# Wuziyi616/multi_part_assembly

Measured on AMD Instinct MI355X. Metric: train-step parts/sec (BxP) at N=1000 pts, higher is better.
Workload: dtype f32

## Files before the change

multi_part_assembly_amd/csrc/pn_bwd_q.h:

```cpp

#ifdef PN_TIMING
#define PN_T_DECL unsigned long long t_busy = 0, t_mark = __builtin_amdgcn_s_memtime(), t_start = t_mark;
#define PN_BAR                                         \
  {                                                    \
    t_busy += __builtin_amdgcn_s_memtime() - t_mark;   \
    __syncthreads();                                   \
    t_mark = __builtin_amdgcn_s_memtime();             \
  }
#define PN_T_REPORT(ROLE)                                                                                              \
  if (blockIdx.x == 5 && lane == 0)                                                                                    \
    printf("K=%d FIRST=%d %s wave %d: units %d busy %llu of %llu cycles\n", K, (int)FIRST, ROLE, wave, n_it, t_busy, \
           __builtin_amdgcn_s_memtime() - t_start);
#else
#define PN_T_DECL
#define PN_BAR __syncthreads();
#define PN_T_REPORT(ROLE)
#endif
#define PN_LDS __attribute__((address_space(3)))
typedef short pn_s16x4 __attribute__((ext_vector_type(4)));
typedef short pn_s16x8 __attribute__((ext_vector_type(8)));
typedef unsigned int pn_u32x4 __attribute__((ext_vector_type(4)));

__device__ __forceinline__ pn_bf16x8 pn_tr_frag(const unsigned char* p, int stride) {
  const pn_s16x4 a = __builtin_amdgcn_ds_read_tr16_b64_v4i16((PN_LDS pn_s16x4*)p);
  const pn_s16x4 b = __builtin_amdgcn_ds_read_tr16_b64_v4i16((PN_LDS pn_s16x4*)(p + 4 * stride));
  const pn_s16x8 v = {a[0], a[1], a[2], a[3], b[0], b[1], b[2], b[3]};
  return __builtin_bit_cast(pn_bf16x8, v);
}

__device__ __forceinline__ void pn_split4(const float v[4], pn_bf16x4& ph, pn_bf16x4& pm, pn_bf16x4& pl) {
#pragma unroll
  for (int u = 0; u < 4; ++u) {
    ph[u] = (__bf16)v[u];
    const float r1 = v[u] - (float)ph[u];
    pm[u] = (__bf16)r1;
    pl[u] = (__bf16)(r1 - (float)pm[u]);
  }
}

typedef float pn_f32x2 __attribute__((ext_vector_type(2)));
typedef __bf16 pn_bf16x2 __attribute__((ext_vector_type(2)));
__device__ __forceinline__ void pn_split2v(pn_f32x2 x, pn_bf16x2& h, pn_bf16x2& m, pn_bf16x2& l) {
  h = __builtin_convertvector(x, pn_bf16x2);
  const pn_f32x2 r = x - __builtin_convertvector(h, pn_f32x2);
  m = __builtin_convertvector(r, pn_bf16x2);
  const pn_f32x2 t = r - __builtin_convertvector(m, pn_f32x2);
  l = __builtin_convertvector(t, pn_bf16x2);
}
__device__ __forceinline__ void pn_split4v(pn_f32x2 a, pn_f32x2 b, pn_bf16x4& ph, pn_bf16x4& pm, pn_bf16x4& pl) {
  pn_bf16x2 h0, m0, l0, h1, m1, l1;
  pn_split2v(a, h0, m0, l0);
  pn_split2v(b, h1, m1, l1);
  ph = pn_bf16x4{h0[0], h0[1], h1[0], h1[1]};
  pm = pn_bf16x4{m0[0], m0[1], m1[0], m1[1]};
  pl = pn_bf16x4{l0[0], l0[1], l1[0], l1[1]};
}

__device__ __forceinline__ void pn_fmac(float& acc, float a, float b) {
  asm volatile("v_fmac_f32 %0, %1, %2" : "+v"(acc) : "v"(a), "v"(b));
}

#define PN_MFMA6(ACC, AH, AM, AL, BH, BM, BL)                          \
  ACC = __builtin_amdgcn_mfma_f32_32x32x16_bf16(AH, BH, ACC, 0, 0, 0); \
  ACC = __builtin_amdgcn_mfma_f32_32x32x16_bf16(AH, BM, ACC, 0, 0, 0); \
  ACC = __builtin_amdgcn_mfma_f32_32x32x16_bf16(AM, BH, ACC, 0, 0, 0); \
  ACC = __builtin_amdgcn_mfma_f32_32x32x16_bf16(AM, BM, ACC, 0, 0, 0); \
  ACC = __builtin_amdgcn_mfma_f32_32x32x16_bf16(AH, BL, ACC, 0, 0, 0); \
  ACC = __builtin_amdgcn_mfma_f32_32x32x16_bf16(AL, BH, ACC, 0, 0, 0);

__global__ void pn_bwd_q_prep_kernel(const float* __restrict__ w, const float* __restrict__ coef, int K, int CIN,
                                     float* __restrict__ q) {
  const int k = blockIdx.x, d = threadIdx.x;
  float acc = 0.0f;
  if (k < CIN) {
#pragma unroll 8
    for (int c = 0; c < K; ++c) acc = __builtin_fmaf(coef[K + c] * w[(long long)c * CIN + k], w[(long long)c * CIN + d], acc);
  } else {
#pragma unroll 8
    for (int c = 0; c < K; ++c) acc = __builtin_fmaf(coef[2 * K + c], w[(long long)c * CIN + d], acc);
  }
  q[(long long)k * CIN + d] = acc;
}

__host__ __device__ constexpr int pn_bwd_q_elems(int K, int CIN, bool first) {
  return K * CIN + CIN * CIN + CIN + (first ? 192 + 12 : 0);
}

template <int N, typename F>
__device__ __forceinline__ void pn_static_for(F&& f) {
  if constexpr (N > 0) {
    pn_static_for<N - 1>(f);
    f(std::integral_constant<int, N - 1>{});
  }
}

struct PnWTile {
  signed char a, b, kind, orow, ocol;
};
template <int K>
struct PnWPlan;
template <>
struct PnWPlan<64> {
  static constexpr int TPW = 2;
  static constexpr PnWTile t[4][2] = {{{0, 8, 0, 0, 0}, {8, 8, 1, 0, 0}},
                                      {{0, 9, 0, 0, 1}, {8, 9, 1, 0, 1}},
                                      {{1, 8, 0, 1, 0}, {-1, -1, 0, 0, 0}},
                                      {{1, 9, 0, 1, 1}, {9, 9, 1, 1, 1}}};
  static constexpr int zc[4] = {0, 0, 1, 1};
  static constexpr bool uses(int w, int code) {
    for (int i = 0; i < TPW; ++i)
      if (t[w][i].a >= 0 && (t[w][i].a == code || t[w][i].b == code)) return true;
    return false;
  }
};
template <>
struct PnWPlan<128> {
  static constexpr int TPW = 3;
  static constexpr PnWTile t[4][3] = {{{0, 8, 0, 0, 0}, {0, 9, 0, 0, 1}, {8, 8, 1, 0, 0}},
                                      {{1, 8, 0, 1, 0}, {1, 9, 0, 1, 1}, {8, 9, 1, 0, 1}},
                                      {{2, 8, 0, 2, 0}, {2, 9, 0, 2, 1}, {9, 9, 1, 1, 1}},
                                      {{3, 8, 0, 3, 0}, {3, 9, 0, 3, 1}, {-1, -1, 0, 0, 0}}};
  static constexpr int zc[4] = {0, 1, 2, 3};
  static constexpr bool uses(int w, int code) {
    for (int i = 0; i < TPW; ++i)
      if (t[w][i].a >= 0 && (t[w][i].a == code || t[w][i].b == code)) return true;
    return false;
  }
};

template <int K, int CIN, int RB, int NS, int ND, int NW, bool FIRST, int KPN = 1>
__global__ __launch_bounds__(64 * (NS + ND + NW), (NS + ND + NW + 3) / 4) void pn_bwd_q_kernel(
    const float* __restrict__ dz, const float* __restrict__ y_prev, const float* __restrict__ bn_prev,
    const float* __restrict__ w, const float* __restrict__ coef, const float* __restrict__ q,
    const int* __restrict__ vlist, int N, float* __restrict__ dz_prev, float* __restrict__ partial,
    float* __restrict__ dwpart, const float* __restrict__ wt1) {
  constexpr int SZ = 6 * K + 16, SA = 6 * CIN + 16;
  constexpr int RT = RB / 32, CT = CIN / 32;
  constexpr int KZ = K / 16, KA = CIN / 16, KW = RB / 16;
  constexpr int NTS = 64 * NS, QK = K / 4, QC = CIN / 4, RG = NTS / QC;
  constexpr int NLZ = RB * QK / NTS, NLY = RB * QC / NTS;
  constexpr int ELEMS = pn_bwd_q_elems(K, CIN, FIRST);
  constexpr int OUTP = RB * CIN;
  static_assert(ND == RT * CT * KPN && RB * QK % NTS == 0 && RB * QC % NTS == 0 && NTS % QK == 0 && NTS % QC == 0, "shapes");
  static_assert(!FIRST || CIN == 64, "the recomputed input is the 64-channel first layer");
  __shared__ __attribute__((aligned(16))) unsigned char pz[2][RB * SZ];
  __shared__ __attribute__((aligned(16))) unsigned char pa[2][RB * SA];
  __shared__ __attribute__((aligned(16))) unsigned char wl[CIN * SZ];
  __shared__ __attribute__((aligned(16))) float outp[2][KPN][OUTP];
  const int wave = __builtin_amdgcn_readfirstlane(threadIdx.x >> 6), lane = threadIdx.x & 63, j = lane & 31, hh = lane >> 5;
  const int TB = (N + RB - 1) / RB, U = vlist[0] * TB, G = gridDim.x;
  const int n_it = (int)blockIdx.x < U ? (U - (int)blockIdx.x + G - 1) / G : 0;
  auto part_of = [&](int it) {
    const int u = (int)blockIdx.x + it * G;
    return u < U && it >= 0 ? vlist[4 + u / TB] : 0;
  };
  auto n0_of = [&](int it) { return (((int)blockIdx.x + it * G) % TB) * RB; };

  for (int e = threadIdx.x; e < CIN * (K / 4); e += blockDim.x) {
    const int d = e % CIN, k4 = e / CIN;
    float v[4];
#pragma unroll
    for (int u = 0; u < 4; ++u) v[u] = coef[4 * k4 + u] * w[(long long)(4 * k4 + u) * CIN + d];
    pn_bf16x4 ph, pm, pl;
    pn_split4(v, ph, pm, pl);
    unsigned char* p = wl + d * SZ + 8 * k4;
    *reinterpret_cast<pn_bf16x4*>(p) = ph;
    *reinterpret_cast<pn_bf16x4*>(p + 2 * K) = pm;
    *reinterpret_cast<pn_bf16x4*>(p + 4 * K) = pl;
  }

  static_assert(NW == NS && ND == NS && NLY % 2 == 0, "the epilogue uses the stagers' thread -> (row, 4 columns) map in both roles");
  constexpr int EH = NLY / 2;
    const int te = threadIdx.x & (NTS - 1);
    const int cy4 = te % QC, ry0 = te / QC;
    const float4 sc = reinterpret_cast<const float4*>(bn_prev)[cy4];
    const float4 sh = reinterpret_cast<const float4*>(bn_prev + CIN)[cy4];
    const float4 mn = reinterpret_cast<const float4*>(bn_prev + 2 * CIN)[cy4];
    float4 w1a = {}, w1b = {}, w1c = {};
    if constexpr (FIRST) {
      w1a = reinterpret_cast<const float4*>(wt1)[cy4];
      w1b = reinterpret_cast<const float4*>(wt1 + 64)[cy4];
      w1c = reinterpret_cast<const float4*>(wt1 + 128)[cy4];
    }
    auto first4 = [&](float4 p) {
      return make_float4(first_layer_y(p.x, p.y, p.z, w1a.x, w1b.x, w1c.x), first_layer_y(p.x, p.y, p.z, w1a.y, w1b.y, w1c.y),
                         first_layer_y(p.x, p.y, p.z, w1a.z, w1b.z, w1c.z), first_layer_y(p.x, p.y, p.z, w1a.w, w1b.w, w1c.w));
    };
    float4 ye[EH];
    float4 s1v = make_float4(0.0f, 0.0f, 0.0f, 0.0f), t2v = s1v;
    float4 sax = s1v, say = s1v, saz = s1v;
    auto load_y = [&](int it, int m, auto half_tag) {
      constexpr int HALF = decltype(half_tag)::value;
      const int n0 = n0_of(it);
      const long long row0 = (long long)m * N + n0;
#pragma unroll
      for (int i = 0; i < EH; ++i) {
        const int rl = ry0 + (HALF * EH + i) * RG;
        const int rr = n0 + rl < N ? rl : N - 1 - n0;
        if constexpr (FIRST) {
          const float* p = y_prev + (row0 + rr) * 3;
          ye[i] = make_float4(p[0], p[1], p[2], 0.0f);
        } else {
          ye[i] = reinterpret_cast<const float4*>(y_prev)[(row0 + rr) * QC + cy4];
        }
      }
    };
    auto epilogue = [&](int it, int m, auto half_tag) {
      constexpr int HALF = decltype(half_tag)::value;
      const int n0 = n0_of(it);
      const long long row0 = (long long)m * N + n0;
      const float* ob = &outp[it & 1][0][0];
#pragma unroll
      for (int i = 0; i < EH; ++i) {
        const int rl = ry0 + (HALF * EH + i) * RG;
        const bool ok = n0 + rl < N;
        float4 o = *reinterpret_cast<const float4*>(ob + rl * CIN + 4 * cy4);
        if constexpr (KPN == 2) {
          const float4 o2 = *reinterpret_cast<const float4*>(ob + OUTP + rl * CIN + 4 * cy4);
          o.x += o2.x;
          o.y += o2.y;
          o.z += o2.z;
          o.w += o2.w;
        }
        float4 yv = ye[i];
        float px = 0.0f, py = 0.0f, pzc = 0.0f;
        if constexpr (FIRST) {
          px = yv.x;
          py = yv.y;
          pzc = yv.z;
          yv = first4(yv);
        }
        float4 d;
        d.x = (ok && __builtin_fmaf(yv.x, sc.x, sh.x) > 0.0f) ? o.x : 0.0f;
        d.y = (ok && __builtin_fmaf(yv.y, sc.y, sh.y) > 0.0f) ? o.y : 0.0f;
        d.z = (ok && __builtin_fmaf(yv.z, sc.z, sh.z) > 0.0f) ? o.z : 0.0f;
        d.w = (ok && __builtin_fmaf(yv.w, sc.w, sh.w) > 0.0f) ? o.w : 0.0f;
        if constexpr (FIRST) {
          sax.x = __builtin_fmaf(d.x, px, sax.x);
          sax.y = __builtin_fmaf(d.y, px, sax.y);
          sax.z = __builtin_fmaf(d.z, px, sax.z);
          sax.w = __builtin_fmaf(d.w, px, sax.w);
          say.x = __builtin_fmaf(d.x, py, say.x);
          say.y = __builtin_fmaf(d.y, py, say.y);
          say.z = __builtin_fmaf(d.z, py, say.z);
          say.w = __builtin_fmaf(d.w, py, say.w);
          saz.x = __builtin_fmaf(d.x, pzc, saz.x);
          saz.y = __builtin_fmaf(d.y, pzc, saz.y);
          saz.z = __builtin_fmaf(d.z, pzc, saz.z);
          saz.w = __builtin_fmaf(d.w, pzc, saz.w);
        } else {
          if (ok) reinterpret_cast<float4*>(dz_prev)[(row0 + rl) * QC + cy4] = d;
        }
        s1v.x += d.x;
        s1v.y += d.y;
        s1v.z += d.z;
        s1v.w += d.w;
        t2v.x = __builtin_fmaf(d.x, yv.x - mn.x, t2v.x);
        t2v.y = __builtin_fmaf(d.y, yv.y - mn.y, t2v.y);
        t2v.z = __builtin_fmaf(d.z, yv.z - mn.z, t2v.z);
        t2v.w = __builtin_fmaf(d.w, yv.w - mn.w, t2v.w);
      }
    };
    auto put_sums = [&](int role) {
      float* scr = reinterpret_cast<float*>(&pz[0][0]);
      const float* isd = bn_prev + 3 * CIN;
      asm volatile("" : "+s"(isd));
      const float4 is4 = reinterpret_cast<const float4*>(isd)[cy4];
      t2v.x *= is4.x;
      t2v.y *= is4.y;
      t2v.z *= is4.z;
      t2v.w *= is4.w;
      *reinterpret_cast<float4*>(scr + ((1 * 2 + role) * RG + ry0) * CIN + 4 * cy4) = s1v;
      *reinterpret_cast<float4*>(scr + ((2 * 2 + role) * RG + ry0) * CIN + 4 * cy4) = t2v;
      if constexpr (FIRST) {
        *reinterpret_cast<float4*>(scr + ((3 * 2 + role) * RG + ry0) * CIN + 4 * cy4) = sax;
        *reinterpret_cast<float4*>(scr + ((4 * 2 + role) * RG + ry0) * CIN + 4 * cy4) = say;
        *reinterpret_cast<float4*>(scr + ((5 * 2 + role) * RG + ry0) * CIN + 4 * cy4) = saz;
      }
    };
    using Half0 = std::integral_constant<int, 0>;
    using Half1 = std::integral_constant<int, 1>;

  if (wave < NS) {
    const int t = threadIdx.x;
    const int cz4 = t % QK, rz0 = t / QK;
    float4 rz[NLZ], ry[NLY];
    float4 colsum = make_float4(0.0f, 0.0f, 0.0f, 0.0f);
    float pp[9] = {0.0f, 0.0f, 0.0f, 0.0f, 0.0f, 0.0f, 0.0f, 0.0f, 0.0f};
    auto load_rows = [&](int it, int m, float4 (&dst)[NLY]) {
      const int n0 = n0_of(it);
      const long long row0 = (long long)m * N + n0;
#pragma unroll
      for (int i = 0; i < NLY; ++i) {
        const int rl = ry0 + i * RG;
        const int rr = n0 + rl < N ? rl : N - 1 - n0;
        if constexpr (FIRST) {
          const float* p = y_prev + (row0 + rr) * 3;
          dst[i] = make_float4(p[0], p[1], p[2], 0.0f);
        } else {
          dst[i] = reinterpret_cast<const float4*>(y_prev)[(row0 + rr) * QC + cy4];
        }
      }
    };
    auto fetch = [&](int it, int m) {
      const int n0 = n0_of(it);
      const long long row0 = (long long)m * N + n0;
#pragma unroll
      for (int i = 0; i < NLZ; ++i) {
        const int rl = rz0 + i * (NTS / QK);
        const int rr = n0 + rl < N ? rl : N - 1 - n0;
        rz[i] = reinterpret_cast<const float4*>(dz)[(row0 + rr) * QK + cz4];
      }
      load_rows(it, m, ry);
    };
    const pn_f32x2 sc01 = {sc.x, sc.y}, sc23 = {sc.z, sc.w}, sh01 = {sh.x, sh.y}, sh23 = {sh.z, sh.w}, zero2 = {0.0f, 0.0f};
    auto stash_t = [&](int it, int b, auto full_tag) {
      constexpr bool FULL = decltype(full_tag)::value;
      const int n0 = n0_of(it);
#pragma unroll
      for (int i = 0; i < NLZ; ++i) {
        const int rl = rz0 + i * (NTS / QK);
        const bool ok = FULL || n0 + rl < N;
        const pn_f32x2 v01 = {ok ? rz[i].x : 0.0f, ok ? rz[i].y : 0.0f}, v23 = {ok ? rz[i].z : 0.0f, ok ? rz[i].w : 0.0f};
        pn_bf16x4 ph, pm, pl;
        pn_split4v(v01, v23, ph, pm, pl);
        unsigned char* p = pz[b] + rl * SZ + 8 * cz4;
        *reinterpret_cast<pn_bf16x4*>(p) = ph;
        *reinterpret_cast<pn_bf16x4*>(p + 2 * K) = pm;
        *reinterpret_cast<pn_bf16x4*>(p + 4 * K) = pl;
      }
#pragma unroll
      for (int i = 0; i < NLY; ++i) {
        const int rl = ry0 + i * RG;
        const bool ok = FULL || n0 + rl < N;
        float4 yv = ry[i];
        if constexpr (FIRST) {
          const float a0 = yv.x, a1 = yv.y, a2 = yv.z;
          if (cy4 == 0 && ok) {
            pn_fmac(pp[0], a0, a0);
            pn_fmac(pp[1], a0, a1);
            pn_fmac(pp[2], a0, a2);
            pn_fmac(pp[3], a1, a1);
            pn_fmac(pp[4], a1, a2);
            pn_fmac(pp[5], a2, a2);
            pn_fmac(pp[6], a0, 1.0f);
            pn_fmac(pp[7], a1, 1.0f);
            pn_fmac(pp[8], a2, 1.0f);
          }
          yv = first4(yv);
        }
        pn_f32x2 v01 = __builtin_elementwise_max(__builtin_elementwise_fma(pn_f32x2{yv.x, yv.y}, sc01, sh01), zero2);
        pn_f32x2 v23 = __builtin_elementwise_max(__builtin_elementwise_fma(pn_f32x2{yv.z, yv.w}, sc23, sh23), zero2);
        if (!ok) v01 = v23 = zero2;
        colsum.x += v01[0];
        colsum.y += v01[1];
        colsum.z += v23[0];
        colsum.w += v23[1];
        pn_bf16x4 ph, pm, pl;
        pn_split4v(v01, v23, ph, pm, pl);
        unsigned char* p = pa[b] + rl * SA + 8 * cy4;
        *reinterpret_cast<pn_bf16x4*>(p) = ph;
        *reinterpret_cast<pn_bf16x4*>(p + 2 * CIN) = pm;
        *reinterpret_cast<pn_bf16x4*>(p + 4 * CIN) = pl;
      }
    };
    auto stash = [&](int it, int b) {
      if (n0_of(it) + RB <= N) stash_t(it, b, std::true_type{});
      else stash_t(it, b, std::false_type{});
    };
    int m2 = part_of(2);
    if (n_it > 0) {
      fetch(0, part_of(0));
      stash(0, 0);
      if (n_it > 1) fetch(1, part_of(1));
    }
    __syncthreads();
    PN_T_DECL
    for (int it = 0; it < n_it; ++it) {
      const int m3 = part_of(it + 3);
      if (it + 1 < n_it) stash(it + 1, (it + 1) & 1);
      if (it + 2 < n_it) fetch(it + 2, m2);
      m2 = m3;
      PN_BAR
    }
    PN_T_REPORT("stager")
    float* scr = reinterpret_cast<float*>(&pz[0][0]);
    *reinterpret_cast<float4*>(scr + (0 * RG + ry0) * CIN + 4 * cy4) = colsum;
    if constexpr (FIRST) {
      if (cy4 == 0) {
#pragma unroll
        for (int e = 0; e < 9; ++e) scr[12 * RG * CIN + ry0 * 12 + e] = pp[e];
      }
    }
  } else if (wave < NS + ND) {
    const int dw = wave - NS, kp = dw % KPN, tile = dw / KPN, rt = tile / CT, ct = tile % CT, d0 = 32 * ct;
    constexpr int KSTEPS = KZ + KA, KPER = KSTEPS / KPN;
    static_assert(KSTEPS % KPN == 0 && (KPN == 1 || KPN == 2), "k-split");
    pn_bf16x8 qh[KA], qm[KA], ql[KA];
#pragma unroll
    for (int ks = 0; ks < KA; ++ks)
#pragma unroll
      for (int u = 0; u < 8; ++u) {
        const float f = q[(long long)(16 * ks + 8 * hh + u) * CIN + d0 + j];
        qh[ks][u] = (__bf16)f;
        const float r1 = f - (float)qh[ks][u];
        qm[ks][u] = (__bf16)r1;
        ql[ks][u] = (__bf16)(r1 - (float)qm[ks][u]);
      }
    const float c0v = kp == KPN - 1 ? q[(long long)CIN * CIN + d0 + j] : 0.0f;
    __syncthreads();
    PN_T_DECL
    int m_prev = 0, m_cur = part_of(0);
    for (int it = 0; it < n_it; ++it) {
      const int b = it & 1;
      const int m_next = part_of(it + 1);
      if (it > 0) epilogue(it - 1, m_prev, Half0{});
      load_y(it, m_cur, Half0{});
      m_prev = m_cur;
      m_cur = m_next;
      f32x16 acc;
#pragma unroll
      for (int r = 0; r < 16; ++r) acc[r] = c0v;
      const unsigned char* arow = pz[b] + (32 * rt + j) * SZ + 16 * hh;
      const unsigned char* brow = wl + (d0 + j) * SZ + 16 * hh;
      const unsigned char* qrow = pa[b] + (32 * rt + j) * SA + 16 * hh;
      auto chain = [&](auto kp_tag) {
        constexpr int LO = decltype(kp_tag)::value * KPER;
        pn_bf16x8 fa[2][3], fb[2][3];
#pragma unroll
        for (int i = 0; i <= KPER; ++i) {
          if (i < KPER) {
            const int ks = LO + i;
            if (ks < KZ) {
#pragma unroll
              for (int pl = 0; pl < 3; ++pl) {
                fa[i & 1][pl] = *reinterpret_cast<const pn_bf16x8*>(arow + 2 * K * pl + 32 * ks);
                fb[i & 1][pl] = *reinterpret_cast<const pn_bf16x8*>(brow + 2 * K * pl + 32 * ks);
              }
            } else {
#pragma unroll
              for (int pl = 0; pl < 3; ++pl)
                fa[i & 1][pl] = *reinterpret_cast<const pn_bf16x8*>(qrow + 2 * CIN * pl + 32 * (ks - KZ));
            }
          }
          if (i > 0) {
            const int ks = LO + i - 1, sb = (i - 1) & 1;
            if (ks < KZ) {
              PN_MFMA6(acc, fa[sb][0], fa[sb][1], fa[sb][2], fb[sb][0], fb[sb][1], fb[sb][2])
            } else {
              PN_MFMA6(acc, fa[sb][0], fa[sb][1], fa[sb][2], qh[ks - KZ], qm[ks - KZ], ql[ks - KZ])
            }
          }
        }
      };
      if (KPN == 1 || kp == 0) chain(std::integral_constant<int, 0>{});
      else chain(std::integral_constant<int, KPN - 1>{});
      float* o = &outp[b][0][0] + kp * OUTP + (32 * rt) * CIN + d0 + j;
#pragma unroll
      for (int r = 0; r < 16; ++r) o[acc_row(r, hh) * CIN] = acc[r];
      PN_BAR
    }
    if (n_it > 0) epilogue(n_it - 1, m_prev, Half0{});
    PN_T_REPORT("dgrad")
    put_sums(0);
  } else {
    const int ww = wave - NS - ND;
    const int g16 = lane >> 4, i16 = lane & 15;
    const int trow = 8 * (g16 >> 1) + (i16 >> 2), tcol = 16 * (g16 & 1) + 4 * (i16 & 3);
    const int offz = trow * SZ + 2 * tcol, offa = trow * SA + 2 * tcol;
    using Plan = PnWPlan<K>;
    static_assert(NW == 4 && CT == 2, "the tile plans are written for four weight-gradient waves and a 64-wide input");
    constexpr int TPW = Plan::TPW;
    f32x16 acc[TPW];
#pragma unroll
    for (int i = 0; i < TPW; ++i) acc[i] = f32x16{0};
    __syncthreads();
    PN_T_DECL
    auto run = [&](auto w_tag) {
      constexpr int W = decltype(w_tag)::value;
      constexpr int ZC = Plan::zc[W];
      constexpr bool A0 = Plan::uses(W, 8), A1 = Plan::uses(W, 9);
      int m_prev = 0, m_cur = part_of(0);
      for (int it = 0; it < n_it; ++it) {
        const int b = it & 1;
        const int m_next = part_of(it + 1);
        if (it > 0) epilogue(it - 1, m_prev, Half1{});
        load_y(it, m_cur, Half1{});
        m_prev = m_cur;
        m_cur = m_next;
        const unsigned char* bz = pz[b] + offz + 64 * ZC;
        const unsigned char* ba = pa[b] + offa;
        pn_bf16x8 fz[2][3], f0[2][3], f1[2][3];
#pragma unroll
        for (int ks = 0; ks <= KW; ++ks) {
          if (ks < KW) {
#pragma unroll
            for (int pl = 0; pl < 3; ++pl) {
              fz[ks & 1][pl] = pn_tr_frag(bz + 16 * ks * SZ + 2 * K * pl, SZ);
              if constexpr (A0) f0[ks & 1][pl] = pn_tr_frag(ba + 16 * ks * SA + 2 * CIN * pl, SA);
              if constexpr (A1) f1[ks & 1][pl] = pn_tr_frag(ba + 16 * ks * SA + 2 * CIN * pl + 64, SA);
            }
          }
          if (ks > 0) {
            const int sb = (ks - 1) & 1;
            pn_static_for<TPW>([&](auto i_tag) {
              constexpr int i = decltype(i_tag)::value;
              constexpr PnWTile t = Plan::t[W][i];
              if constexpr (t.a >= 0) {
                const pn_bf16x8(&fa)[3] = *(t.a < 8 ? &fz[sb] : (t.a == 8 ? &f0[sb] : &f1[sb]));
                const pn_bf16x8(&fb)[3] = *(t.b == 8 ? &f0[sb] : &f1[sb]);
                PN_MFMA6(acc[i], fa[0], fa[1], fa[2], fb[0], fb[1], fb[2])
              }
            });
          }
        }
        PN_BAR
      }
      if (n_it > 0) epilogue(n_it - 1, m_prev, Half1{});
      float* out = dwpart + (long long)blockIdx.x * ELEMS;
      pn_static_for<TPW>([&](auto i_tag) {
        constexpr int i = decltype(i_tag)::value;
        constexpr PnWTile t = Plan::t[W][i];
        if constexpr (t.a >= 0) {
          float* o = out + (t.kind == 0 ? 0 : K * CIN);
#pragma unroll
          for (int r = 0; r < 16; ++r) o[(32 * t.orow + acc_row(r, hh)) * CIN + 32 * t.ocol + j] = acc[i][r];
        }
      });
    };
    if (ww == 0) run(std::integral_constant<int, 0>{});
    else if (ww == 1) run(std::integral_constant<int, 1>{});
    else if (ww == 2) run(std::integral_constant<int, 2>{});
    else run(std::integral_constant<int, 3>{});
    PN_T_REPORT("wgrad")
    put_sums(1);
  }
  __syncthreads();
  {
    const float* scr = reinterpret_cast<const float*>(&pz[0][0]);
    float* out = dwpart + (long long)blockIdx.x * ELEMS;
    const int t = threadIdx.x;
    constexpr int NQ = FIRST ? 6 : 3;
    if (t < NQ * CIN) {
      const int qq = t / CIN, c = t % CIN;
      float s = 0.0f;
#pragma unroll
      for (int g = 0; g < (qq == 0 ? 1 : 2) * RG; ++g) s += scr[(qq * 2 * RG + g) * CIN + c];
      if (qq == 0) out[K * CIN + CIN * CIN + c] = s;
      else if (qq <= 2) partial[((long long)blockIdx.x * CIN + c) * 2 + (qq - 1)] = s;
      else out[K * CIN + CIN * CIN + CIN + 3 * c + (qq - 3)] = s;
    } else if (FIRST && t < NQ * CIN + 9) {
      const int e = t - NQ * CIN;
      float s = 0.0f;
#pragma unroll
      for (int g = 0; g < RG; ++g) s += scr[12 * RG * CIN + g * 12 + e];
      out[K * CIN + CIN * CIN + CIN + 192 + e] = s;
    }
  }
}

struct PnGTile {
  signed char a, b;
};
struct PnGPlan {
  static constexpr int TPW = 3;
  static constexpr PnGTile t[4][3] = {{{0, 0}, {0, 1}, {0, 2}}, {{1, 1}, {1, 2}, {1, 3}}, {{0, 3}, {3, 3}, {-1, -1}}, {{2, 2}, {2, 3}, {-1, -1}}};
  static constexpr bool uses(int w, int tile) {
    for (int i = 0; i < TPW; ++i)
      if (t[w][i].a >= 0 && (t[w][i].a == tile || t[w][i].b == tile)) return true;
    return false;
  }
};

template <int CIN, int NS, int ND, int NW>
__global__ __launch_bounds__(64 * (NS + ND + NW), (NS + ND + NW + 3) / 4) void pn_bwd_top_q_kernel(
    const float* __restrict__ y_prev, const float* __restrict__ bn_prev, const float* __restrict__ q,
    const int* __restrict__ vlist, int N, float* __restrict__ dz_prev, float* __restrict__ partial,
    float* __restrict__ dwpart, const int2* __restrict__ rtile, const float* __restrict__ rsum, int F) {
  constexpr int K = 0;
  constexpr bool FIRST = false;
  constexpr int RB = 32, SA = 6 * CIN + 16, CT = CIN / 32, KA = CIN / 16, KW = RB / 16;
  constexpr int NTS = 64 * NS, QC = CIN / 4, RG = NTS / QC, NLY = RB * QC / NTS;
  constexpr int ELEMS = CIN * CIN + CIN;
  static_assert(CIN == 128 && ND == CT && NW == 4 && NS == 4 && NLY % 2 == 0, "shapes");
  __shared__ __attribute__((aligned(16))) unsigned char pa[2][RB * SA];
  __shared__ __attribute__((aligned(16))) float outp[2][RB * CIN];
  __shared__ __attribute__((aligned(16))) float rowsum[3][RB * CIN];
  const int wave = __builtin_amdgcn_readfirstlane(threadIdx.x >> 6), lane = threadIdx.x & 63, j = lane & 31, hh = lane >> 5;
  const int TB = (N + RB - 1) / RB, U = vlist[0] * TB, G = gridDim.x;
  const int n_it = (int)blockIdx.x < U ? (U - (int)blockIdx.x + G - 1) / G : 0;
  auto part_of = [&](int it) {
    const int u = (int)blockIdx.x + it * G;
    return u < U && it >= 0 ? vlist[4 + u / TB] : 0;
  };
  auto n0_of = [&](int it) { return (((int)blockIdx.x + it * G) % TB) * RB; };

  if (wave < NS) {
    const int te = threadIdx.x;
    int cy4 = te % QC, ry0 = te / QC;
    const float4 sc = reinterpret_cast<const float4*>(bn_prev)[cy4];
    const float4 sh = reinterpret_cast<const float4*>(bn_prev + CIN)[cy4];
    const float4 mn = reinterpret_cast<const float4*>(bn_prev + 2 * CIN)[cy4];
    const int T1 = (N + 31) / 32 + 1;
    float4 ya[NLY], yb[NLY], yc[NLY];
    float4 colsum = make_float4(0.0f, 0.0f, 0.0f, 0.0f);
    float4 s1v = colsum, t2v = colsum;
    const pn_f32x2 sc01 = {sc.x, sc.y}, sc23 = {sc.z, sc.w}, sh01 = {sh.x, sh.y}, sh23 = {sh.z, sh.w}, zero2 = {0.0f, 0.0f};
    auto fetch = [&](int it, int m, float4(&ry)[NLY]) {
      const int n0 = n0_of(it);
      const long long row0 = (long long)m * N + n0;
#pragma unroll
      for (int i = 0; i < NLY; ++i) {
        const int rl = ry0 + i * RG;
        const int rr = n0 + rl < N ? rl : N - 1 - n0;
        ry[i] = reinterpret_cast<const float4*>(y_prev)[(row0 + rr) * QC + cy4];
      }
    };
    auto stash = [&](int it, int b, const float4(&ry)[NLY]) {
      const int n0 = n0_of(it);
#pragma unroll
      for (int i = 0; i < NLY; ++i) {
        const int rl = ry0 + i * RG;
        const bool ok = n0 + rl < N;
        pn_f32x2 v01 = __builtin_elementwise_max(__builtin_elementwise_fma(pn_f32x2{ry[i].x, ry[i].y}, sc01, sh01), zero2);
        pn_f32x2 v23 = __builtin_elementwise_max(__builtin_elementwise_fma(pn_f32x2{ry[i].z, ry[i].w}, sc23, sh23), zero2);
        if (!ok) v01 = v23 = zero2;
        colsum.x += v01[0];
        colsum.y += v01[1];
        colsum.z += v23[0];
        colsum.w += v23[1];
        pn_bf16x4 ph, pm, pl;
        pn_split4v(v01, v23, ph, pm, pl);
        unsigned char* p = pa[b] + rl * SA + 8 * cy4;
        *reinterpret_cast<pn_bf16x4*>(p) = ph;
        *reinterpret_cast<pn_bf16x4*>(p + 2 * CIN) = pm;
        *reinterpret_cast<pn_bf16x4*>(p + 4 * CIN) = pl;
      }
    };
    auto epilogue = [&](int it, int m, const float4(&ye)[NLY]) {
      const int n0 = n0_of(it), slot = it % 3;
      const auto dzr = __builtin_amdgcn_make_buffer_rsrc(dz_prev + ((long long)m * N + n0) * CIN, 0,
                                                         (N - n0 < RB ? N - n0 : RB) * CIN * 4, 0x00020000);
      const float* ob = &outp[it & 1][0];
#pragma unroll
      for (int i = 0; i < NLY; ++i) {
        const int rl = ry0 + i * RG;
        const bool ok = n0 + rl < N;
        float4 o = *reinterpret_cast<const float4*>(ob + rl * CIN + 4 * cy4);
        const float4 sp = *reinterpret_cast<const float4*>(&rowsum[slot][rl * CIN + 4 * cy4]);
        o.x += sp.x;
        o.y += sp.y;
        o.z += sp.z;
        o.w += sp.w;
        const float4 yv = ye[i];
        float4 d;
        d.x = (ok && __builtin_fmaf(yv.x, sc.x, sh.x) > 0.0f) ? o.x : 0.0f;
        d.y = (ok && __builtin_fmaf(yv.y, sc.y, sh.y) > 0.0f) ? o.y : 0.0f;
        d.z = (ok && __builtin_fmaf(yv.z, sc.z, sh.z) > 0.0f) ? o.z : 0.0f;
        d.w = (ok && __builtin_fmaf(yv.w, sc.w, sh.w) > 0.0f) ? o.w : 0.0f;
        __builtin_amdgcn_raw_buffer_store_b128(__builtin_bit_cast(pn_u32x4, d), dzr, (rl * CIN + 4 * cy4) * 4, 0, 0);
        s1v.x += d.x;
        s1v.y += d.y;
        s1v.z += d.z;
        s1v.w += d.w;
        t2v.x = __builtin_fmaf(d.x, yv.x - mn.x, t2v.x);
        t2v.y = __builtin_fmaf(d.y, yv.y - mn.y, t2v.y);
        t2v.z = __builtin_fmaf(d.z, yv.z - mn.z, t2v.z);
        t2v.w = __builtin_fmaf(d.w, yv.w - mn.w, t2v.w);
      }
    };
    int2 rt = make_int2(0, 0);
    float4 rv[NLY];
    auto rt_fetch = [&](int it, int m) { rt = rtile[(long long)m * T1 + (n0_of(it) >> 5)]; };
    auto rows_fetch = [&](int m) {
      const int bytes = F * CIN * 4;
      const auto rsr = __builtin_amdgcn_make_buffer_rsrc(const_cast<float*>(rsum) + (long long)m * F * CIN, 0, bytes, 0x00020000);
#pragma unroll
      for (int i = 0; i < NLY; ++i) {
        const int rl = ry0 + i * RG;
        const unsigned mask = (unsigned)rt.y;
        const int jr = rt.x + __builtin_popcount(mask & ((1u << rl) - 1u));
        rv[i] = __builtin_bit_cast(float4, __builtin_amdgcn_raw_buffer_load_b128(rsr, (mask >> rl) & 1u ? (jr * CIN + 4 * cy4) * 4 : bytes, 0, 0));
      }
    };
    auto rows_stash = [&](int it) {
      const int slot = it % 3;
#pragma unroll
      for (int i = 0; i < NLY; ++i) *reinterpret_cast<float4*>(&rowsum[slot][(ry0 + i * RG) * CIN + 4 * cy4]) = rv[i];
    };
    int m1 = part_of(1), m2 = part_of(2), m3 = part_of(3);
    int m_prev = 0, m_cur = part_of(0);
    if (n_it > 0) {
      rt_fetch(0, m_cur);
      fetch(0, m_cur, yb);
      rows_fetch(m_cur);
      if (n_it > 1) rt_fetch(1, m1);
      rows_stash(0);
      stash(0, 0, yb);
      if (n_it > 1) {
        fetch(1, m1, yc);
        rows_fetch(m1);
      }
      if (n_it > 2) rt_fetch(2, m2);
    }
    __syncthreads();
    PN_T_DECL
    auto step = [&](int it, auto steady_tag) {
      constexpr bool STEADY = decltype(steady_tag)::value;
      const int m4 = part_of(it + 4);
      asm volatile("" : "+v"(cy4), "+v"(ry0));
      if (STEADY || it > 0) epilogue(it - 1, m_prev, ya);
      if (STEADY || it + 1 < n_it) rows_stash(it + 1);
#pragma unroll
      for (int i = 0; i < NLY; ++i) {
        ya[i] = yb[i];
        yb[i] = yc[i];
      }
      if (STEADY || it + 2 < n_it) {
        fetch(it + 2, m2, yc);
        rows_fetch(m2);
      }
      if (STEADY || it + 3 < n_it) rt_fetch(it + 3, m3);
      if (STEADY || it + 1 < n_it) stash(it + 1, (it + 1) & 1, yb);
      m_prev = m_cur;
      m_cur = m1;
      m1 = m2;
      m2 = m3;
      m3 = m4;
      PN_BAR
    };
    int it = 0;
    for (int phase = 0; phase < 2; ++phase) {
      const int hi = phase == 0 ? (n_it < 1 ? n_it : 1) : n_it;
      for (; it < hi; ++it) step(it, std::false_type{});
      if (phase == 0)
        for (; it + 3 < n_it; ++it) step(it, std::true_type{});
    }
    if (n_it > 0) epilogue(n_it - 1, m_prev, ya);
    PN_T_REPORT("stager")
    float* scr = reinterpret_cast<float*>(&pa[0][0]);
    const float4 is4 = reinterpret_cast<const float4*>(bn_prev + 3 * CIN)[cy4];
    t2v.x *= is4.x;
    t2v.y *= is4.y;
    t2v.z *= is4.z;
    t2v.w *= is4.w;
    *reinterpret_cast<float4*>(scr + (0 * RG + ry0) * CIN + 4 * cy4) = colsum;
    *reinterpret_cast<float4*>(scr + (1 * RG + ry0) * CIN + 4 * cy4) = s1v;
    *reinterpret_cast<float4*>(scr + (2 * RG + ry0) * CIN + 4 * cy4) = t2v;
  } else if (wave < NS + ND) {
    const int ct = wave - NS, d0 = 32 * ct;
    pn_bf16x8 qh[KA], qm[KA], ql[KA];
#pragma unroll
    for (int ks = 0; ks < KA; ++ks)
#pragma unroll
      for (int u = 0; u < 8; ++u) {
        const float f = q[(long long)(16 * ks + 8 * hh + u) * CIN + d0 + j];
        qh[ks][u] = (__bf16)f;
        const float r1 = f - (float)qh[ks][u];
        qm[ks][u] = (__bf16)r1;
        ql[ks][u] = (__bf16)(r1 - (float)qm[ks][u]);
      }
    const float c0v = q[(long long)CIN * CIN + d0 + j];
    __syncthreads();
    PN_T_DECL
    for (int it = 0; it < n_it; ++it) {
      const int b = it & 1;
      f32x16 acc;
#pragma unroll
      for (int r = 0; r < 16; ++r) acc[r] = c0v;
      const unsigned char* qrow = pa[b] + j * SA + 16 * hh;
      pn_bf16x8 fa[2][3];
#pragma unroll
      for (int i = 0; i <= KA; ++i) {
        if (i < KA) {
#pragma unroll
          for (int pl = 0; pl < 3; ++pl) fa[i & 1][pl] = *reinterpret_cast<const pn_bf16x8*>(qrow + 2 * CIN * pl + 32 * i);
        }
        if (i > 0) {
          const int sb = (i - 1) & 1;
          PN_MFMA6(acc, fa[sb][0], fa[sb][1], fa[sb][2], qh[i - 1], qm[i - 1], ql[i - 1])
        }
      }
      float* o = &outp[b][0] + d0 + j;
#pragma unroll
      for (int r = 0; r < 16; ++r) o[acc_row(r, hh) * CIN] = acc[r];
      PN_BAR
    }
    PN_T_REPORT("dgrad")
  } else {
    const int ww = wave - NS - ND;
    const int g16 = lane >> 4, i16 = lane & 15;
    const int trow = 8 * (g16 >> 1) + (i16 >> 2), tcol = 16 * (g16 & 1) + 4 * (i16 & 3);
    const int offa = trow * SA + 2 * tcol;
    constexpr int TPW = PnGPlan::TPW;
    f32x16 acc[TPW];
#pragma unroll
    for (int i = 0; i < TPW; ++i) acc[i] = f32x16{0};
    __syncthreads();
    PN_T_DECL
    auto run = [&](auto w_tag) {
      constexpr int W = decltype(w_tag)::value;
      for (int it = 0; it < n_it; ++it) {
        const unsigned char* ba = pa[it & 1] + offa;
        pn_bf16x8 f[4][3];
#pragma unroll
        for (int ks = 0; ks < KW; ++ks) {
          pn_static_for<4>([&](auto c_tag) {
            constexpr int c = decltype(c_tag)::value;
            if constexpr (PnGPlan::uses(W, c)) {
#pragma unroll
              for (int pl = 0; pl < 3; ++pl) f[c][pl] = pn_tr_frag(ba + 16 * ks * SA + 2 * CIN * pl + 64 * c, SA);
            }
          });
          pn_static_for<TPW>([&](auto i_tag) {
            constexpr int i = decltype(i_tag)::value;
            constexpr PnGTile tl = PnGPlan::t[W][i];
            if constexpr (tl.a >= 0) {
              PN_MFMA6(acc[i], f[tl.a][0], f[tl.a][1], f[tl.a][2], f[tl.b][0], f[tl.b][1], f[tl.b][2])
            }
          });
        }
        PN_BAR
      }
      float* out = dwpart + (long long)blockIdx.x * ELEMS;
      pn_static_for<TPW>([&](auto i_tag) {
        constexpr int i = decltype(i_tag)::value;
        constexpr PnGTile tl = PnGPlan::t[W][i];
        if constexpr (tl.a >= 0) {
#pragma unroll
          for (int r = 0; r < 16; ++r) {
            const int ra = 32 * tl.a + acc_row(r, hh), cb = 32 * tl.b + j;
            out[ra * CIN + cb] = acc[i][r];
            if (tl.a != tl.b) out[cb * CIN + ra] = acc[i][r];
          }
        }
      });
    };
    if (ww == 0) run(std::integral_constant<int, 0>{});
    else if (ww == 1) run(std::integral_constant<int, 1>{});
    else if (ww == 2) run(std::integral_constant<int, 2>{});
    else run(std::integral_constant<int, 3>{});
    PN_T_REPORT("gram")
  }
  __syncthreads();
  {
    const float* scr = reinterpret_cast<const float*>(&pa[0][0]);
    float* out = dwpart + (long long)blockIdx.x * ELEMS;
    const int t = threadIdx.x;
    if (t < 3 * CIN) {
      const int qq = t / CIN, c = t % CIN;
      float s = 0.0f;
#pragma unroll
      for (int g = 0; g < RG; ++g) s += scr[(qq * RG + g) * CIN + c];
      if (qq == 0) out[CIN * CIN + c] = s;
      else partial[((long long)blockIdx.x * CIN + c) * 2 + (qq - 1)] = s;
    }
  }
}

struct PnFinish {
  const float* red[3];
  const float* w[3];
  const float* coef[3];
  float* dw[3];
  int K[3], CIN[3], first[4];
  const float* w1;
  const float* coef1;
  float* dw1;
  int first_layer;
};
__global__ __launch_bounds__(256) void pn_bwd_finish_kernel(const PnFinish f) {
  if ((int)blockIdx.x == f.first[3]) {
    const int t = threadIdx.x;
    if (t >= 192) return;
    const int c = t / 3, k = t % 3, i = f.first_layer;
    const float* x = f.red[i] + f.K[i] * f.CIN[i] + f.CIN[i] * f.CIN[i] + f.CIN[i];
    const float* pp = x + 192;
    float wg = 0.0f;
#pragma unroll
    for (int jx = 0; jx < 3; ++jx) {
      const int a = jx < k ? jx : k, b = jx < k ? k : jx;
      wg = __builtin_fmaf(f.w1[c * 3 + jx], pp[a == 0 ? b : (a == 1 ? 2 + b : 5)], wg);
    }
    f.dw1[t] = f.coef1[c] * x[t] + f.coef1[64 + c] * wg + f.coef1[128 + c] * pp[6 + k];
    return;
  }
  int i = 0;
#pragma unroll
  for (int qq = 1; qq < 3; ++qq) i += (int)blockIdx.x >= f.first[qq] ? 1 : 0;
  const int K = f.K[i], CIN = f.CIN[i];
  const int e = ((int)blockIdx.x - f.first[i]) * 256 + threadIdx.x;
  if (e >= K * CIN) return;
  const int c = e / CIN, d = e % CIN;
  const float* T = f.red[i];
  const float* Gm = T + K * CIN;
  const float* asum = Gm + CIN * CIN;
  const float* wr = f.w[i] + (long long)c * CIN;
  float wg = 0.0f;
#pragma unroll 8
  for (int k = 0; k < CIN; ++k) {
    const float g = (k >> 5) <= (d >> 5) ? Gm[k * CIN + d] : Gm[d * CIN + k];
    wg = __builtin_fmaf(wr[k], g, wg);
  }
  f.dw[i][e] = f.coef[i][c] * T[e] + f.coef[i][K + c] * wg + f.coef[i][2 * K + c] * asum[d];
}
```

Before: 376,100.

## Deepen stager prefetch to two in-flight tiles and replace per-iteration div/mod indexing

The stager waves now keep two register buffers of dz/y rows in flight, fetching two units ahead and unrolling the loop by two so global loads overlap more barriers. Per-iteration part and row-offset computation, which used integer division and modulo, is replaced by an incremental (part, tile) cursor in all three wave roles. Compiler barriers and waitcnt hints pin register liveness and scheduling. The first-layer moment accumulation becomes branchless. This costs more VGPRs in the stagers and adds complex tail handling, which risks lower occupancy or off-by-one errors.

Measured after the change: 366,400. 0.974x the previous value.

```diff
diff --git a/multi_part_assembly_amd/csrc/pn_bwd_q.h b/multi_part_assembly_amd/csrc/pn_bwd_q.h
--- a/multi_part_assembly_amd/csrc/pn_bwd_q.h
+++ b/multi_part_assembly_amd/csrc/pn_bwd_q.h
@@ -20,6 +20,8 @@
 typedef short pn_s16x4 __attribute__((ext_vector_type(4)));
 typedef short pn_s16x8 __attribute__((ext_vector_type(8)));
 typedef unsigned int pn_u32x4 __attribute__((ext_vector_type(4)));
+typedef float pn_f32x4 __attribute__((ext_vector_type(4)));
+typedef float pn_f32x3 __attribute__((ext_vector_type(3)));
 
 __device__ __forceinline__ pn_bf16x8 pn_tr_frag(const unsigned char* p, int stride) {
   const pn_s16x4 a = __builtin_amdgcn_ds_read_tr16_b64_v4i16((PN_LDS pn_s16x4*)p);
@@ -150,11 +152,16 @@
   const int wave = __builtin_amdgcn_readfirstlane(threadIdx.x >> 6), lane = threadIdx.x & 63, j = lane & 31, hh = lane >> 5;
   const int TB = (N + RB - 1) / RB, U = vlist[0] * TB, G = gridDim.x;
   const int n_it = (int)blockIdx.x < U ? (U - (int)blockIdx.x + G - 1) / G : 0;
-  auto part_of = [&](int it) {
-    const int u = (int)blockIdx.x + it * G;
-    return u < U && it >= 0 ? vlist[4 + u / TB] : 0;
+  const int NP = vlist[0], dpi = G / TB, dtl = G % TB;
+  auto advance = [&](int& pi, int& tl) {
+    tl += dtl;
+    pi += dpi;
+    if (tl >= TB) {
+      tl -= TB;
+      ++pi;
+    }
   };
-  auto n0_of = [&](int it) { return (((int)blockIdx.x + it * G) % TB) * RB; };
+  auto part_at = [&](int pi) { return vlist[4 + (pi < NP ? pi : NP - 1)]; };
 
   for (int e = threadIdx.x; e < CIN * (K / 4); e += blockDim.x) {
     const int d = e % CIN, k4 = e / CIN;
@@ -172,7 +179,7 @@
   static_assert(NW == NS && ND == NS && NLY % 2 == 0, "the epilogue uses the stagers' thread -> (row, 4 columns) map in both roles");
   constexpr int EH = NLY / 2;
     const int te = threadIdx.x & (NTS - 1);
-    const int cy4 = te % QC, ry0 = te / QC;
+    int cy4 = te % QC, ry0 = te / QC;
     const float4 sc = reinterpret_cast<const float4*>(bn_prev)[cy4];
     const float4 sh = reinterpret_cast<const float4*>(bn_prev + CIN)[cy4];
     const float4 mn = reinterpret_cast<const float4*>(bn_prev + 2 * CIN)[cy4];
@@ -189,9 +196,8 @@
     float4 ye[EH];
     float4 s1v = make_float4(0.0f, 0.0f, 0.0f, 0.0f), t2v = s1v;
     float4 sax = s1v, say = s1v, saz = s1v;
-    auto load_y = [&](int it, int m, auto half_tag) {
+    auto load_y = [&](int n0, int m, auto half_tag) {
       constexpr int HALF = decltype(half_tag)::value;
-      const int n0 = n0_of(it);
       const long long row0 = (long long)m * N + n0;
 #pragma unroll
       for (int i = 0; i < EH; ++i) {
@@ -205,11 +211,10 @@
         }
       }
     };
-    auto epilogue = [&](int it, int m, auto half_tag) {
+    auto epilogue = [&](int n0, int m, int b, auto half_tag) {
       constexpr int HALF = decltype(half_tag)::value;
-      const int n0 = n0_of(it);
       const long long row0 = (long long)m * N + n0;
-      const float* ob = &outp[it & 1][0][0];
+      const float* ob = &outp[b][0][0];
 #pragma unroll
       for (int i = 0; i < EH; ++i) {
         const int rl = ry0 + (HALF * EH + i) * RG;
@@ -282,41 +287,37 @@
     using Half1 = std::integral_constant<int, 1>;
 
   if (wave < NS) {
+    __builtin_amdgcn_s_waitcnt(0x0F70);
     const int t = threadIdx.x;
     const int cz4 = t % QK, rz0 = t / QK;
-    float4 rz[NLZ], ry[NLY];
+    using YRow = std::conditional_t<FIRST, pn_f32x3, pn_f32x4>;
+    pn_f32x4 za[NLZ], zb[NLZ];
+    YRow ya[NLY], yb[NLY];
     float4 colsum = make_float4(0.0f, 0.0f, 0.0f, 0.0f);
     float pp[9] = {0.0f, 0.0f, 0.0f, 0.0f, 0.0f, 0.0f, 0.0f, 0.0f, 0.0f};
-    auto load_rows = [&](int it, int m, float4 (&dst)[NLY]) {
-      const int n0 = n0_of(it);
+    auto fetch = [&](int n0, int m, pn_f32x4 (&rz)[NLZ], YRow (&ry)[NLY]) {
       const long long row0 = (long long)m * N + n0;
+#pragma unroll
+      for (int i = 0; i < NLZ; ++i) {
+        const int rl = rz0 + i * (NTS / QK);
+        const int rr = n0 + rl < N ? rl : N - 1 - n0;
+        rz[i] = reinterpret_cast<const pn_f32x4*>(dz)[(row0 + rr) * QK + cz4];
+      }
 #pragma unroll
       for (int i = 0; i < NLY; ++i) {
         const int rl = ry0 + i * RG;
         const int rr = n0 + rl < N ? rl : N - 1 - n0;
         if constexpr (FIRST) {
           const float* p = y_prev + (row0 + rr) * 3;
-          dst[i] = make_float4(p[0], p[1], p[2], 0.0f);
+          ry[i] = pn_f32x3{p[0], p[1], p[2]};
         } else {
-          dst[i] = reinterpret_cast<const float4*>(y_prev)[(row0 + rr) * QC + cy4];
-        }
-      }
-    };
-    auto fetch = [&](int it, int m) {
-      const int n0 = n0_of(it);
-      const long long row0 = (long long)m * N + n0;
-#pragma unroll
-      for (int i = 0; i < NLZ; ++i) {
-        const int rl = rz0 + i * (NTS / QK);
-        const int rr = n0 + rl < N ? rl : N - 1 - n0;
-        rz[i] = reinterpret_cast<const float4*>(dz)[(row0 + rr) * QK + cz4];
-      }
-      load_rows(it, m, ry);
+          ry[i] = reinterpret_cast<const pn_f32x4*>(y_prev)[(row0 + rr) * QC + cy4];
+        }
+      }
     };
     const pn_f32x2 sc01 = {sc.x, sc.y}, sc23 = {sc.z, sc.w}, sh01 = {sh.x, sh.y}, sh23 = {sh.z, sh.w}, zero2 = {0.0f, 0.0f};
-    auto stash_t = [&](int it, int b, auto full_tag) {
+    auto stash_t = [&](int n0, int b, const pn_f32x4 (&rz)[NLZ], const YRow (&ry)[NLY], auto full_tag) {
       constexpr bool FULL = decltype(full_tag)::value;
-      const int n0 = n0_of(it);
 #pragma unroll
       for (int i = 0; i < NLZ; ++i) {
         const int rl = rz0 + i * (NTS / QK);
@@ -333,19 +334,22 @@
       for (int i = 0; i < NLY; ++i) {
         const int rl = ry0 + i * RG;
         const bool ok = FULL || n0 + rl < N;
-        float4 yv = ry[i];
+        float4 yv;
+        if constexpr (FIRST) yv = make_float4(ry[i].x, ry[i].y, ry[i].z, 0.0f);
+        else yv = make_float4(ry[i].x, ry[i].y, ry[i].z, ry[i].w);
         if constexpr (FIRST) {
           const float a0 = yv.x, a1 = yv.y, a2 = yv.z;
-          if (cy4 == 0 && ok) {
-            pn_fmac(pp[0], a0, a0);
-            pn_fmac(pp[1], a0, a1);
-            pn_fmac(pp[2], a0, a2);
-            pn_fmac(pp[3], a1, a1);
-            pn_fmac(pp[4], a1, a2);
-            pn_fmac(pp[5], a2, a2);
-            pn_fmac(pp[6], a0, 1.0f);
-            pn_fmac(pp[7], a1, 1.0f);
-            pn_fmac(pp[8], a2, 1.0f);
+          {
+            const float b0 = ok ? a0 : 0.0f, b1 = ok ? a1 : 0.0f, b2 = ok ? a2 : 0.0f;
+            pn_fmac(pp[0], b0, a0);
+            pn_fmac(pp[1], b0, a1);
+            pn_fmac(pp[2], b0, a2);
+            pn_fmac(pp[3], b1, a1);
+            pn_fmac(pp[4], b1, a2);
+            pn_fmac(pp[5], b2, a2);
+            pn_fmac(pp[6], b0, 1.0f);
+            pn_fmac(pp[7], b1, 1.0f);
+            pn_fmac(pp[8], b2, 1.0f);
           }
           yv = first4(yv);
         }
@@ -364,25 +368,77 @@
         *reinterpret_cast<pn_bf16x4*>(p + 4 * CIN) = pl;
       }
     };
-    auto stash = [&](int it, int b) {
-      if (n0_of(it) + RB <= N) stash_t(it, b, std::true_type{});
-      else stash_t(it, b, std::false_type{});
-    };
-    int m2 = part_of(2);
+    auto stash = [&](int n0, int b, const pn_f32x4 (&rz)[NLZ], const YRow (&ry)[NLY]) {
+      if (n0 + RB <= N) stash_t(n0, b, rz, ry, std::true_type{});
+      else stash_t(n0, b, rz, ry, std::false_type{});
+    };
+    int pi = (int)blockIdx.x / TB, tl = (int)blockIdx.x % TB;
+    int n0f = tl * RB, mf = part_at(pi);
+    advance(pi, tl);
+    int m_nx = part_at(pi);
+    auto next_unit = [&]() {
+      n0f = tl * RB;
+      mf = m_nx;
+      advance(pi, tl);
+      m_nx = part_at(pi);
+    };
+    int n0a = 0, n0b = 0;
     if (n_it > 0) {
-      fetch(0, part_of(0));
-      stash(0, 0);
-      if (n_it > 1) fetch(1, part_of(1));
+      n0b = n0f;
+      fetch(n0f, mf, zb, yb);
+      next_unit();
+      if (n_it > 1) {
+        n0a = n0f;
+        fetch(n0f, mf, za, ya);
+        next_unit();
+      }
+      stash(n0b, 0, zb, yb);
+      if (n_it > 2) {
+        n0b = n0f;
+        fetch(n0f, mf, zb, yb);
+        next_unit();
+      } else {
+        __builtin_amdgcn_s_waitcnt(0x0F70);
+      }
     }
     __syncthreads();
     PN_T_DECL
-    for (int it = 0; it < n_it; ++it) {
-      const int m3 = part_of(it + 3);
-      if (it + 1 < n_it) stash(it + 1, (it + 1) & 1);
-      if (it + 2 < n_it) fetch(it + 2, m2);
-      m2 = m3;
+    auto arrive = [&](pn_f32x4 (&rz)[NLZ], YRow (&ry)[NLY]) {
+#pragma unroll
+      for (int i = 0; i < NLZ; ++i) asm volatile("" : "+v"(rz[i]));
+#pragma unroll
+      for (int i = 0; i < NLY; ++i) asm volatile("" : "+v"(ry[i]));
+    };
+    int it = 0;
+    for (; it + 4 < n_it; it += 2) {
+      arrive(za, ya);
+      stash(n0a, 1, za, ya);
+      n0a = n0f;
+      fetch(n0f, mf, za, ya);
+      next_unit();
       PN_BAR
-    }
+      arrive(zb, yb);
+      stash(n0b, 0, zb, yb);
+      n0b = n0f;
+      fetch(n0f, mf, zb, yb);
+      next_unit();
+      PN_BAR
+    }
+    if (it < n_it) {
+      if (it + 1 < n_it) stash(n0a, 1, za, ya);
+      if (it + 3 < n_it) fetch(n0f, mf, za, ya);
+      n0a = n0f;
+      PN_BAR
+    }
+    if (it + 1 < n_it) {
+      if (it + 2 < n_it) stash(n0b, 0, zb, yb);
+      PN_BAR
+    }
+    if (it + 2 < n_it) {
+      if (it + 3 < n_it) stash(n0a, 1, za, ya);
+      PN_BAR
+    }
+    if (it + 3 < n_it) PN_BAR
     PN_T_REPORT("stager")
     float* scr = reinterpret_cast<float*>(&pz[0][0]);
     *reinterpret_cast<float4*>(scr + (0 * RG + ry0) * CIN + 4 * cy4) = colsum;
@@ -408,16 +464,21 @@
         ql[ks][u] = (__bf16)(r1 - (float)qm[ks][u]);
       }
     const float c0v = kp == KPN - 1 ? q[(long long)CIN * CIN + d0 + j] : 0.0f;
+#pragma unroll
+    for (int ks = 0; ks < KA; ++ks) asm volatile("" : "+v"(qh[ks]), "+v"(qm[ks]), "+v"(ql[ks]));
     __syncthreads();
     PN_T_DECL
-    int m_prev = 0, m_cur = part_of(0);
+    int pi = (int)blockIdx.x / TB, tl = (int)blockIdx.x % TB;
+    int n0_prev = 0, m_prev = 0, n0_cur = tl * RB, m_cur = part_at(pi);
+    advance(pi, tl);
+    int m_nx = part_at(pi);
     for (int it = 0; it < n_it; ++it) {
       const int b = it & 1;
-      const int m_next = part_of(it + 1);
-      if (it > 0) epilogue(it - 1, m_prev, Half0{});
-      load_y(it, m_cur, Half0{});
-      m_prev = m_cur;
-      m_cur = m_next;
+      asm volatile("" ::"s"(m_nx));
+      if constexpr (FIRST) asm volatile("" : "+v"(cy4), "+v"(ry0));
+      if (it > 0) epilogue(n0_prev, m_prev, b ^ 1, Half0{});
+      load_y(n0_cur, m_cur, Half0{});
+      if constexpr (FIRST) __builtin_amdgcn_sched_barrier(0);
       f32x16 acc;
 #pragma unroll
       for (int r = 0; r < 16; ++r) acc[r] = c0v;
@@ -458,9 +519,16 @@
       float* o = &outp[b][0][0] + kp * OUTP + (32 * rt) * CIN + d0 + j;
 #pragma unroll
       for (int r = 0; r < 16; ++r) o[acc_row(r, hh) * CIN] = acc[r];
+      n0_prev = n0_cur;
+      m_prev = m_cur;
+      n0_cur = tl * RB;
+      m_cur = m_nx;
+      advance(pi, tl);
+      asm volatile("" : "+s"(pi));
+      m_nx = part_at(pi);
       PN_BAR
     }
-    if (n_it > 0) epilogue(n_it - 1, m_prev, Half0{});
+    if (n_it > 0) epilogue(n0_prev, m_prev, (n_it - 1) & 1, Half0{});
     PN_T_REPORT("dgrad")
     put_sums(0);
   } else {
@@ -480,14 +548,16 @@
       constexpr int W = decltype(w_tag)::value;
       constexpr int ZC = Plan::zc[W];
       constexpr bool A0 = Plan::uses(W, 8), A1 = Plan::uses(W, 9);
-      int m_prev = 0, m_cur = part_of(0);
+      int pi = (int)blockIdx.x / TB, tl = (int)blockIdx.x % TB;
+      int n0_prev = 0, m_prev = 0, n0_cur = tl * RB, m_cur = part_at(pi);
+      advance(pi, tl);
+      int m_nx = part_at(pi);
       for (int it = 0; it < n_it; ++it) {
         const int b = it & 1;
-        const int m_next = part_of(it + 1);
-        if (it > 0) epilogue(it - 1, m_prev, Half1{});
-        load_y(it, m_cur, Half1{});
-        m_prev = m_cur;
-        m_cur = m_next;
+        asm volatile("" ::"s"(m_nx));
+        if constexpr (FIRST) asm volatile("" : "+v"(cy4), "+v"(ry0));
+        if (it > 0) epilogue(n0_prev, m_prev, b ^ 1, Half1{});
+        load_y(n0_cur, m_cur, Half1{});
         const unsigned char* bz = pz[b] + offz + 64 * ZC;
         const unsigned char* ba = pa[b] + offa;
         pn_bf16x8 fz[2][3], f0[2][3], f1[2][3];
@@ -514,9 +584,16 @@
             });
           }
         }
+        n0_prev = n0_cur;
+        m_prev = m_cur;
+        n0_cur = tl * RB;
+        m_cur = m_nx;
+        advance(pi, tl);
+        asm volatile("" : "+s"(pi));
+        m_nx = part_at(pi);
         PN_BAR
       }
-      if (n_it > 0) epilogue(n_it - 1, m_prev, Half1{});
+      if (n_it > 0) epilogue(n0_prev, m_prev, (n_it - 1) & 1, Half1{});
       float* out = dwpart + (long long)blockIdx.x * ELEMS;
       pn_static_for<TPW>([&](auto i_tag) {
         constexpr int i = decltype(i_tag)::value;
```
